# YufengJin/BundleSDF

Hardware: AMD Instinct MI355X
Metric: NeRF training rays/sec + ms/iter, 64-frame pool, 2048 rays/frame (higher is better)
Workload: dtype fp16 table+MLP (MFMA) / fp32 accumulate+Adam (amp)

## Files before the change

### bundlesdf_amd/csrc/field_step.hip

```cpp
#include <algorithm>
#include <cstdlib>
#include <cstring>
#include <array>
#include <type_traits>
#include <vector>

#include "nof_device.h"
#include "ray_trace.h"
#include "mlp_lds.h"

#pragma clang fp contract(off)

#ifndef NOF_ABLATE
#define NOF_ABLATE 0
#endif
#define ABL(bits) (NOF_ABLATE && (a.ablate & (bits)))
#define ABL_HOST(d, bits) (NOF_ABLATE && ((d)->ablate & (bits)))
#define ABL_SKIPQ(q) ((q) < 2 ? (1 << (23 + (q))) : (1 << (27 + (q))))

namespace nof {

typedef _Float16 h8v __attribute__((ext_vector_type(8)));
typedef float f16v __attribute__((ext_vector_type(16)));

constexpr int MLP_N_MAX = 9107 + 64 * 3;
struct MlpOff {
    int w1, b1, w2, b2, w3, b3, w4, b4, w5, b5, n, in, cin;
    __host__ __device__ MlpOff(int IN, int FF = 0) : in(IN), cin(24 + FF) {
        w1 = 0; b1 = 64 * IN; w2 = b1 + 64; b2 = w2 + 16 * 64; w3 = b2 + 16; b3 = w3 + 64 * cin; w4 = b3 + 64;
        b4 = w4 + 64 * 64; w5 = b4 + 64; b5 = w5 + 3 * 64; n = b5 + 3;
    }
};
constexpr int FR_L1 = 0, FR_L2 = 4, FR_L3 = 8, FR_L4 = 12, FR_L5 = 20, FR_B5 = 24, FR_B4 = 26, FR_B3 = 34,
              FR_B2 = 38, FR_B1 = 42, N_FRAGS = 46;
__device__ __forceinline__ int cin_col(int i, int ff) {
    return (i >= 1 && i <= 15) ? ff + 9 + i - 1
                               : ((i >= 16 && i <= 24) ? ff + i - 16 : ((i >= 25 && i < 25 + ff) ? i - 25 : -1));
}
constexpr float SH_C0 = 0.28209479177387814f, SH_C1 = 0.4886025119029199f;
constexpr float SH_C2_0 = 1.0925484305920792f, SH_C2_1 = -1.0925484305920792f, SH_C2_2 = 0.31539156525252005f,
                SH_C2_3 = -1.0925484305920792f, SH_C2_4 = 0.5462742152960396f;

struct FieldArgs {
    const float *rays;
    const float *tf;
    const float *intervals;
    const float *totals;
    float *rctx;
    const float *t_rand;
    uint32_t seed;
    int R, Kmax, N_oct, N_dep, S;
    int perturb;
    float near_sc, far_sc, trunc, ntr, lambda, fs_sdf, ffw, rgb_w, fs_w, empty_w, trunc_w;
    float fs_rgb_w;
    float inv_3R, inv_RS, inv_3RS;
    const float *loss_scale;
    const void *table;
    const float4 *levels;
    uint32_t L;
    int mlp_in;
    int n_ff;
    const float *ff;
    float *grad_ff;
    const void *frags;
    const float *bias;
    float *grad_table;
    __half *grad_table16;
    float *grad_mlp;
    float *ray_grad;
    uint32_t *tile_gmask;
    const uint4 *quads;
    uint32_t n_rows;
    bool quads_ready;
    float *loss_part;
    float *loss_acc;
    float *dbg_z;
    float *dbg_raw;
    uint8_t *dbg_valid;
    float *dbg_rgb;
    void *feat;
    void *dfeat;
    float *zbuf;
    uint8_t *tile_bwd;
    uint32_t slot_mask;
    int *tile_sid;
    int *n_tiles;
    float *ray_aux;
    float4 *tile_aux;
    int ablate;
    int xcd_order;
    const nof_step_params *sp;
    int no_dx;
    int scatter_lpw;
    float *rrec;
    int *ctile_list;
    int bwd_flush;
    int count_atomics;
    int compact_per;
    int encode_group;
};

constexpr int LOSS_ACC_COUNTERS = 136;
constexpr int LOSS_ACC_WORDS = 144;
constexpr int TREC = 12;
enum { TR_WSUM = 0, TR_NVALID, TR_LFS, TR_LEM, TR_LSDF, TR_CNT, TR_RACC = 8, TR_LFSR = 11 };
enum { TC_SIG = 1, TC_COL = 2, TC_CRCOL = 4, TC_CRSIG = 8 };
constexpr int LOSS_COPIES = 64, LOSS_SLOTS = 16, LOSS_FOLD_N = 13;
constexpr uint64_t LOSS_ZERO_WORDS = 16 + (uint64_t)LOSS_COPIES * LOSS_SLOTS;

__device__ __forceinline__ FieldArgs step_args(const FieldArgs &a0) {
    FieldArgs a = a0;
    if (a0.sp) {
        a.trunc = a0.sp->trunc;
        a.seed = a0.sp->seed;
    }
    return a;
}

__device__ __forceinline__ const FieldArgs &late_args() {
    auto k = __builtin_amdgcn_kernarg_segment_ptr();
    asm volatile("" : "+s"(k));
    return *(const FieldArgs *)k;
}

__device__ __forceinline__ int acc_row(int q, int h) { return (q & 3) + 8 * (q >> 2) + 4 * h; }

template <int CTRL, int ROWS = 0xf>
__device__ __forceinline__ float dpp_add(float v) {
    return v + __builtin_bit_cast(float, __builtin_amdgcn_update_dpp(0, __builtin_bit_cast(int, v), CTRL, ROWS, 0xf, true));
}
__device__ __forceinline__ float row_prefix(float v) {
    v = dpp_add<0x111>(v);
    v = dpp_add<0x112>(v);
    v = dpp_add<0x114>(v);
    return dpp_add<0x118>(v);
}
__device__ __forceinline__ float lane_value(float v, int l) {
    return __builtin_bit_cast(float, __builtin_amdgcn_readlane(__builtin_bit_cast(int, v), l));
}
__device__ __forceinline__ float wave_sum(float v) {
    v = row_prefix(v);
    v = dpp_add<0x142, 0xa>(v);
    v = dpp_add<0x143, 0xc>(v);
    return lane_value(v, 63);
}
__device__ __forceinline__ void half_sums(float v, float &s0, float &s1) {
    v = row_prefix(v);
    v = dpp_add<0x142, 0xa>(v);
    s0 = lane_value(v, 31);
    s1 = lane_value(v, 63);
}

__device__ __forceinline__ float sigmoidf(float x) { return __builtin_amdgcn_rcpf(1.0f + __expf(-x)); }
__device__ __forceinline__ int xcd_block(int b, int nb) {
    const int per = nb >> 3, rem = nb & 7, x = b & 7, i = b >> 3;
    return (x < rem ? x * (per + 1) : rem * (per + 1) + (x - rem) * per) + i;
}

__device__ __forceinline__ uint32_t hash32(uint32_t x) {
    x ^= x >> 16; x *= 0x7feb352dU; x ^= x >> 15; x *= 0x846ca68bU; x ^= x >> 16;
    return x;
}
__device__ __forceinline__ float rng_uniform(uint32_t seed, uint32_t ray, uint32_t s) {
    uint32_t h = hash32(seed ^ hash32(ray * 0x9E3779B1U + hash32(s + 0x632BE5ABU)));
    return (float)(h >> 8) * (1.0f / 16777216.0f);
}

__device__ __forceinline__ float linspace01(int i, int n) {
    if (n == 1) return 0.0f;
    const float step = 1.0f / (float)(n - 1);
    return (i < n / 2) ? __builtin_fmaf(step, (float)i, 0.0f) : __builtin_fmaf(-step, (float)(n - 1 - i), 1.0f);
}

template <typename TM> struct FragT;
template <> struct FragT<_Float16> { typedef h8v T; };
template <> struct FragT<float> { struct T { float v[8]; }; };

template <typename TM> __device__ __forceinline__ void frag_set(typename FragT<TM>::T &f, int j, float x);
template <> __device__ __forceinline__ void frag_set<_Float16>(h8v &f, int j, float x) { f[j] = (_Float16)x; }
template <> __device__ __forceinline__ void frag_set<float>(FragT<float>::T &f, int j, float x) { f.v[j] = x; }
template <typename TM> __device__ __forceinline__ float frag_get(const typename FragT<TM>::T &f, int j);
template <> __device__ __forceinline__ float frag_get<_Float16>(const h8v &f, int j) { return (float)f[j]; }
// ... 977 lines not shown
#pragma unroll
        for (int d = 0; d < 3; ++d) {
            pos[k][d] = __builtin_fmaf(x01[d], li.scale, 0.5f);
            pg[d] = (uint32_t)pos[k][d];
            pos[k][d] = __builtin_amdgcn_fractf(pos[k][d]);
        }
        base[k] = dense_base_v(li.off, pg, rs[k]);
    }
    typedef typename std::conditional<sizeof(TT) == 4, float4, uint2>::type Raw;
    Raw raw[G][4];
    const __amdgpu_buffer_rsrc_t trs = table_rsrc(a.table);
    if constexpr (sizeof(TT) == 2) {
        if (a.quads) {
            const __amdgpu_buffer_rsrc_t qrs = table_rsrc(a.quads);
#pragma unroll
            for (int k = 0; k < G; ++k) {
                const uint32_t b0 = dense[k] ? base[k] : 0u, b1 = dense[k] ? base[k] + rs2[k] : 0u;
                const u4v q0 = __builtin_amdgcn_raw_buffer_load_b128(qrs, b0 * 16u, 0, 0);
                const u4v q1 = __builtin_amdgcn_raw_buffer_load_b128(qrs, b1 * 16u, 0, 0);
                raw[k][0] = make_uint2(q0.x, q0.y);
                raw[k][1] = make_uint2(q0.z, q0.w);
                raw[k][2] = make_uint2(q1.x, q1.y);
                raw[k][3] = make_uint2(q1.z, q1.w);
            }
            goto sums;
        }
    }
#pragma unroll
    for (int k = 0; k < G; ++k)
#pragma unroll
        for (int i = 0; i < 4; ++i) {
            raw[k][i] = Raw{};
            if (dense[k]) {
                const uint32_t row = base[k] + ((i & 1) ? rs[k] : 0u) + ((i & 2) ? rs2[k] : 0u);
                if constexpr (sizeof(TT) == 4) {
                    const TT *ptr = tab + (size_t)row * 2;
                    typedef float f4a __attribute__((ext_vector_type(4), aligned(8)));
                    const f4a v = *reinterpret_cast<const f4a *>(ptr);
                    raw[k][i] = make_float4(v.x, v.y, v.z, v.w);
                } else {
                    raw[k][i] = table_pair16(trs, row);
                }
            }
        }
sums:
#pragma unroll
    for (int k = 0; k < G; ++k) {
        out[k][0] = 0.f;
        out[k][1] = 0.f;
        if (!(on && lvs[k] < (int)a.L)) continue;
        if (!dense[k]) {
            encode_level<TT>(a, lis[k], x01, out[k]);
            continue;
        }
        if constexpr (sizeof(TT) == 2) {
            float o0 = 0.f, o1 = 0.f;
#pragma unroll
            for (int idx = 0; idx < 8; ++idx) {
                float w = 1.f;
#pragma unroll
                for (int d = 0; d < 3; ++d) w *= ((idx >> d) & 1) ? pos[k][d] : 1 - pos[k][d];
                const uint32_t pr = (idx & 1) ? raw[k][idx >> 1].y : raw[k][idx >> 1].x;
                asm("v_fma_mix_f32 %0, %1, %2, %0 op_sel_hi:[0,1,0]" : "+v"(o0) : "v"(w), "v"(pr));
                asm("v_fma_mix_f32 %0, %1, %2, %0 op_sel:[0,1,0] op_sel_hi:[0,1,0]" : "+v"(o1) : "v"(w), "v"(pr));
            }
            out[k][0] = o0;
            out[k][1] = o1;
        } else {
            float e[8][2];
#pragma unroll
            for (int i = 0; i < 4; ++i) {
                e[2 * i][0] = raw[k][i].x; e[2 * i][1] = raw[k][i].y;
                e[2 * i + 1][0] = raw[k][i].z; e[2 * i + 1][1] = raw[k][i].w;
            }
#pragma unroll
            for (int idx = 0; idx < 8; ++idx) {
                float w = 1.f;
#pragma unroll
                for (int d = 0; d < 3; ++d) w *= ((idx >> d) & 1) ? pos[k][d] : 1 - pos[k][d];
                out[k][0] = __builtin_fmaf(w, e[idx][0], out[k][0]);
                out[k][1] = __builtin_fmaf(w, e[idx][1], out[k][1]);
            }
        }
    }
}

template <typename TM, typename TT, int G, bool DBG>
__global__ __launch_bounds__(512) __attribute__((amdgpu_num_sgpr(80),
                                                 amdgpu_waves_per_eu(sizeof(TM) == 2 ? (G == 1 ? 8 : G == 2 ? 6 : 4) : (G == 4 ? 4 : 5), 8)))
void k_encode(FieldArgs a_) {
    const FieldArgs a = step_args(a_);
    const int lane = threadIdx.x & 63, n = lane & 31, h = lane >> 5;
    const int ntiles = a.S / 32;
    constexpr int WPB = 8;
    extern __shared__ __attribute__((aligned(16))) char smem[];
    {
        typedef __attribute__((address_space(1))) void *GPtr;
        typedef __attribute__((address_space(3))) void *LPtr;
        const int wv = threadIdx.x >> 6;
        if (ABL(16)) {
            const uint4 *src = reinterpret_cast<const uint4 *>(a.frags);
            uint4 *dst = reinterpret_cast<uint4 *>(smem);
            for (int i = threadIdx.x; i < 8 * 64 * 8 * (int)sizeof(TM) / 16; i += blockDim.x) dst[i] = src[i];
            float *s_b = reinterpret_cast<float *>(smem + 8 * 64 * 8 * sizeof(TM));
            for (int i = threadIdx.x; i < 2 * 64; i += blockDim.x) s_b[i] = a.bias[i];
            __syncthreads();
        } else {
#pragma unroll
            for (int i = 0; i < (int)sizeof(TM) / 2; ++i) {
                const size_t off = (size_t)i * 8192 + (size_t)wv * 1024;
                __builtin_amdgcn_global_load_lds((GPtr)((const char *)a.frags + off + lane * 16), (LPtr)(smem + off), 16,
                                                 0, 0);
            }
            if (wv < 2)
                __builtin_amdgcn_global_load_lds((GPtr)(a.bias + wv * 64 + lane),
                                                 (LPtr)(smem + 8 * 64 * 8 * sizeof(TM) + wv * 256), 4, 0, 0);
        }
    }
    uint4 *lvt = reinterpret_cast<uint4 *>(smem + 8 * 64 * 8 * sizeof(TM) + 2 * 64 * sizeof(float)) + (threadIdx.x >> 6) * 32;
    level_table(a, lvt, lane);
    const int bx = (a.xcd_order & 1) ? xcd_block(blockIdx.x, gridDim.x) : (int)blockIdx.x;
    const int gw0 = __builtin_amdgcn_readfirstlane(bx * WPB + (int)(threadIdx.x >> 6));
    const bool in_range = gw0 < a.R * ntiles;
    const int gw = in_range ? gw0 : a.R * ntiles - 1;
    const int r = gw / ntiles, t = gw - r * ntiles;
    if (ABL(1 << 19)) return;
    const RayCtx c = load_ray(a, r);
    const int s = 32 * t + n;
    const size_t sid = (size_t)r * a.S + s;
    float z = sample_z(a, r, s, c.depth, c.vdepth, c.total, c.box);
    if (ABL(4)) {
        const float z2 = sample_z(a, r, s, c.depth * 0.999f, c.vdepth, c.total * 0.999f, c.box);
        z = z2 == 12345.f ? z2 : z;
    }
    float p[3], x[3];
    const bool valid = sample_point(c, z, p, x);
    if (h == 0 && in_range) {
        a.zbuf[sid] = z;
        if (DBG && a.dbg_z) a.dbg_z[sid] = z;
        if (DBG && a.dbg_valid) a.dbg_valid[sid] = valid;
    }
    if (ABL(8192)) return;
    const float x01[3] = {(x[0] + 1) / 2, (x[1] + 1) / 2, (x[2] + 1) / 2};
    typename FragT<TM>::T f[2];
#pragma unroll
    for (int g0 = 0; g0 < 8; g0 += G) {
        int lvs[G];
#pragma unroll
        for (int k = 0; k < G; ++k) lvs[k] = lane_level((g0 + k) >> 2, (g0 + k) & 3, h);
        float v[G][2];
        encode_levels<TT, G, true, true>(a, lvs, valid && !ABL(8), x01, v, lvt);
#pragma unroll
        for (int k = 0; k < G; ++k) {
            frag_set<TM>(f[(g0 + k) >> 2], 2 * ((g0 + k) & 3), v[k][0]);
            frag_set<TM>(f[(g0 + k) >> 2], 2 * ((g0 + k) & 3) + 1, v[k][1]);
        }
    }
    {
        if (!ABL(64)) __syncthreads();
        if (!in_range) return;
        const FieldArgs a = step_args(late_args());
        const bool tvalid = __any(valid);
        uint8_t *flag = a.tile_bwd + (size_t)r * ntiles + t;
        float4 *trec = reinterpret_cast<float4 *>(a.rrec + ((size_t)r * ntiles + t) * TREC);
        float ws = 0.f, nv = 0.f;
        if (!ABL(2)) half_sums(h == 0 ? bell_weight(a, c.depth, z) : (valid ? 1.f : 0.f), ws, nv);
        if (!tvalid && !(DBG && a.dbg_raw)) {
            if (lane == 0) {
                *flag = 0;
                if (trec) {
                    trec[0] = make_float4(ws, nv, 0.f, 0.f);
                    trec[1] = make_float4(0.f, 0.f, 0.f, 0.f);
                }
            }
            return;
        }
        const TM *s_fr = reinterpret_cast<const TM *>(smem);
        const float *s_b = reinterpret_cast<const float *>(smem + 8 * 64 * 8 * sizeof(TM));
        Acts<TM> A;
        A.X[0] = f[0];
        A.X[1] = f[1];
        float sdf = 0.f;
        f16v l2;
        if (ABL(256)) {
#pragma unroll
            for (int q = 0; q < 16; ++q) l2[q] = 0.f;
            sdf = z * 1e-3f;
        } else {
            mlp_sdf_net<TM>(LdsWt<TM>(s_fr, lane), s_b, A, lane, sdf, l2);
        }
        const float w = bell_weight(a, c.depth, z);
        const bool front = z < c.depth - a.trunc;
        const bool fsr = a.fs_rgb_w > 0.f && front && valid && c.rtype == 0;
        const bool colour = __any(w > 0.f && valid) || __any(fsr) || (DBG && a.dbg_raw != nullptr);
        const float sv = valid ? 1.f : 0.f;
        const bool back = z > c.depth + a.trunc * a.ntr;
        const float sdfm = (!front && !back && c.vdepth) ? 1.f : 0.f;
        const bool fsm = (c.depth > a.far_sc) && (sdf < a.fs_sdf);
        const bool em = front && (c.depth <= a.far_sc) && (sdf < 1.f);
        const float efs = fsm ? (sdf - a.fs_sdf) : 0.f;
        const float esdf = (z + sdf * a.trunc) * sdfm - c.depth * sdfm;
        float dsdf = a.fs_w * 0.5f * 2.f * efs * sv * a.inv_RS;
        dsdf += em ? a.fs_w * a.empty_w * (sdf > 1.f ? 1.f : (sdf < 1.f ? -1.f : 0.f)) * sv * a.inv_RS : 0.f;
        dsdf += a.trunc_w * 0.5f * 2.f * esdf * sdfm * a.trunc * sv * a.inv_RS;
        const bool cand = tvalid && c.rtype == 0 && (__any(w > 0.f && valid) || __any(dsdf != 0.f) || __any(fsr));
        if (lane == 0) *flag = cand ? (colour ? 1 : 2) : (colour ? 3 : 0);
        if (trec && !ABL(2)) {
            float lfs = 0.f, lem = 0.f, lsd = 0.f;
            if (__any(dsdf != 0.f)) {
                half_sums(h == 0 ? a.fs_w * 0.5f * efs * efs * sv * a.inv_RS
                                 : (em ? a.fs_w * a.empty_w * fabsf(sdf - 1.f) * sv * a.inv_RS : 0.f),
                          lfs, lem);
                float unused;
                half_sums(h == 0 ? a.trunc_w * 0.5f * esdf * esdf * sv * a.inv_RS : 0.f, lsd, unused);
            }
            if (lane == 0) {
                const int cnt = TC_SIG | (colour ? TC_COL : 0) | (cand ? (colour ? TC_CRCOL : TC_CRSIG) : 0);
                trec[0] = make_float4(ws, nv, lfs, lem);
                trec[1] = make_float4(lsd, __int_as_float(cnt), 0.f, 0.f);
            }
            if (DBG && a.dbg_raw && h == 0) a.dbg_raw[(((size_t)r * ntiles + t) * 32 + n) * 4 + 3] = sdf;
        }
        const size_t slot = (size_t)r * ntiles + t;
        if (ABL(32768)) return;
        if (cand) {
            store_chunk<TM>(a.feat, (size_t)r * a.S + 32 * t, n, 0, h, f[0]);
            store_chunk<TM>(a.feat, (size_t)r * a.S + 32 * t, n, 1, h, f[1]);
            if (h == 0) a.tile_aux[slot * TILE_AUX + 64 + n] = make_float4(dsdf, valid ? w : 0.f, sv, fsr ? 1.f : 0.f);
            const uint32_t gmask = (uint32_t)__ballot(h == 0 && valid && (w > 0.f || dsdf != 0.f || fsr));
            if (lane == 0) a.tile_gmask[slot] = gmask;
        }
        if (colour) {
            typename FragT<TM>::T cin;
            acc_to_frag<TM>(l2, 0, false, cin);
            store_cin<TM>(a.tile_aux + slot * TILE_AUX, lane, cin);
        }
    }
}

template <typename TM>
__device__ __forceinline__ void stage_mlp(const FieldArgs &a, char *smem) {
    TM *s_fr = reinterpret_cast<TM *>(smem);
    float *s_b = reinterpret_cast<float *>(smem + N_FRAGS * 64 * 8 * sizeof(TM));
    const uint4 *src = reinterpret_cast<const uint4 *>(a.frags);
// ... 803 lines not shown
}
}

namespace {
struct FieldWorkspace {
    size_t feat, dfeat, zbuf, tile_bwd, tile_sid, n_tiles, ray_aux, tile_aux, rctx, gmask, rrec, ctile, total;
    FieldWorkspace(int R, int S, int mlp_dtype) {
        auto al = [](size_t b) { return (b + 255) & ~(size_t)255; };
        const size_t el = mlp_dtype == NOF_F16 ? 2 : 4, n = (size_t)R * S, nt = (size_t)R * (S / 32);
        size_t o = 0;
        feat = o; o += al(n * 32 * el);
        dfeat = o; o += al(n * 32 * el);
        zbuf = o; o += al(n * 4);
        tile_bwd = o; o += al(nt);
        tile_sid = o; o += al(nt * 4);
        n_tiles = o; o += al(4 * nof::LOSS_ZERO_WORDS);
        ray_aux = o; o += al((size_t)R * nof::RAY_AUX * 4);
        tile_aux = o; o += al(nt * nof::TILE_AUX * 16);
        rctx = o; o += al((size_t)R * nof::RCTX * 4);
        gmask = o; o += al(nt * 4);
        rrec = o; o += al(nt * nof::TREC * 4);
        ctile = o; o += al(nt * 4);
        total = o;
    }
};
}

extern "C" size_t nof_field_workspace_bytes(int32_t R, int32_t S, int32_t mlp_dtype) {
    return FieldWorkspace(R, S, mlp_dtype).total;
}

extern "C" int nof_field_workspace_offsets(int32_t R, int32_t S, int32_t mlp_dtype, uint64_t *offsets, int32_t n) {
    if (R < 0 || S <= 0 || !offsets || n < NOF_WS_SECTIONS)
        return nof::set_error(NOF_EINVAL, "field_workspace_offsets: bad R=%d S=%d or n=%d < %d", R, S, n,
                              NOF_WS_SECTIONS);
    const FieldWorkspace w(R, S, mlp_dtype);
    const size_t o[NOF_WS_SECTIONS] = {w.feat, w.dfeat, w.zbuf, w.tile_bwd, w.tile_sid, w.n_tiles, w.ray_aux,
                                       w.tile_aux, w.rctx, w.gmask, w.rrec, w.ctile, w.total};
    for (int i = 0; i < NOF_WS_SECTIONS; ++i) offsets[i] = o[i];
    return NOF_OK;
}

namespace {
bool quads_on(const nof_field_desc *d) {
    return d->table_quads && d->table_rows > 0 && d->mlp_dtype == NOF_F16 && d->table_dtype == NOF_F16 &&
           d->R >= (d->quads_min_rays > 0 ? d->quads_min_rays : 32768) && !ABL_HOST(d, 512);
}
int cu_count() {
    int dev = 0, n_cu = 256;
    if (hipGetDevice(&dev) != hipSuccess ||
        hipDeviceGetAttribute(&n_cu, hipDeviceAttributeMultiprocessorCount, dev) != hipSuccess)
        n_cu = 256;
    return n_cu;
}
}

extern "C" size_t nof_field_desc_size(void) { return sizeof(nof_field_desc); }

extern "C" int nof_quad_mirror(const nof_field_desc *d, void *stream) {
    if (d->L > 16 || d->C != 2)
        return nof::set_error(NOF_EINVAL, "quad_mirror: needs C=2, L<=16 (got %u,%u)", d->C, d->L);
    if (d->R <= 0 || !quads_on(d)) return NOF_OK;
    nof::FieldArgs a{};
    a.table = d->table; a.levels = (const float4 *)d->levels; a.L = d->L;
    a.quads = (const uint4 *)d->table_quads; a.n_rows = (uint32_t)d->table_rows;
    const int n_cu = cu_count();
    hipLaunchKernelGGL(nof::k_quad_mirror, dim3((int)std::min<int64_t>((int64_t)n_cu * 8, nof::div_up(a.n_rows, 256))),
                       dim3(256), 0, (hipStream_t)stream, a);
    return nof::check_launch("quad_mirror");
}

extern "C" int nof_field_step(const nof_field_desc *d, void *stream) {
    if (d->S % 32 != 0 || d->S > 320 || d->N_oct + d->N_dep != d->S)
        return nof::set_error(NOF_EINVAL, "field_step: S=%d must be N_oct+N_dep, a multiple of 32, <= 320", d->S);
    if (d->L > 16 || d->C != 2 || d->D != 3)
        return nof::set_error(NOF_EINVAL, "field_step: needs D=3, C=2, L<=16 (got %u,%u,%u)", d->D, d->C, d->L);
    if (d->R <= 0) return NOF_OK;
    if (d->bwd_flush < 0 || d->bwd_flush > 2)
        return nof::set_error(NOF_EINVAL, "field_step: bwd_flush %d (0 by batch size, 1 per wave, 2 block)", d->bwd_flush);
    if (d->compact_per_block != 0 && (d->compact_per_block < 256 || d->compact_per_block > nof::COMPACT_PER_BLOCK ||
                                      d->compact_per_block % 256 != 0))
        return nof::set_error(NOF_EINVAL, "field_step: compact_per_block %d (0 by batch size, else a multiple of 256 "
                              "in [256, %d])", d->compact_per_block, nof::COMPACT_PER_BLOCK);
    if (d->encode_group != 0 && d->encode_group != 1 && d->encode_group != 2 && d->encode_group != 4)
        return nof::set_error(NOF_EINVAL, "field_step: encode_group %d (0 by batch size, or 1, 2, 4)", d->encode_group);
    if (d->n_ff < 0 || d->n_ff > 3 || (d->n_ff > 0 && (!d->ff || !d->grad_ff)))
        return nof::set_error(NOF_EINVAL, "field_step: frame_features must be 0..3 with ff and grad_ff set (got %d)",
                              d->n_ff);
    if (d->mlp_dtype == NOF_F16 && !d->grad_table16)
        return nof::set_error(NOF_EINVAL, "field_step: amp mode needs grad_table16 (fp16 table gradient)");
    if (d->ablate && !NOF_ABLATE)
        return nof::set_error(NOF_EINVAL, "field_step: ablate bits need a -DNOF_ABLATE=1 build (timing experiments only)");
    if (!d->workspace) return nof::set_error(NOF_EINVAL, "field_step: workspace is NULL (nof_field_workspace_bytes)");
    const int slots = d->scatter_slots ? d->scatter_slots : 512;
    if (slots < 64 || slots > 2048 || (slots & (slots - 1)))
        return nof::set_error(NOF_EINVAL, "field_step: scatter_slots must be a power of two in [64, 2048]");
    const bool amp = d->mlp_dtype == NOF_F16 && d->table_dtype == NOF_F16;
    if (!amp && !(d->mlp_dtype == NOF_F32 && d->table_dtype == NOF_F32))
        return nof::set_error(NOF_EINVAL, "field_step: mlp/table dtype must both be f16 (amp) or both f32");

    nof::FieldArgs a;
    a.rays = d->rays; a.tf = d->tf; a.intervals = d->intervals; a.totals = d->totals; a.t_rand = d->t_rand;
    a.seed = d->seed; a.R = d->R; a.Kmax = d->Kmax; a.N_oct = d->N_oct; a.N_dep = d->N_dep; a.S = d->S;
    a.perturb = d->perturb; a.near_sc = d->near_sc; a.far_sc = d->far_sc; a.trunc = d->trunc;
    a.ntr = d->neg_trunc_ratio; a.lambda = d->sdf_lambda; a.fs_sdf = d->fs_sdf; a.ffw = d->first_frame_weight;
    a.rgb_w = d->rgb_weight; a.fs_w = d->fs_weight; a.empty_w = d->empty_weight; a.trunc_w = d->trunc_weight;
    a.inv_3R = 1.0f / (3.0f * (float)d->R);
    a.inv_RS = 1.0f / ((float)d->R * (float)d->S);
    a.inv_3RS = 1.0f / (3.0f * (float)d->R * (float)d->S);
    a.xcd_order = d->xcd_order;
    a.no_dx = d->skip_pose_grad != 0;
    a.quads = quads_on(d) ? (const uint4 *)d->table_quads : nullptr;
    a.n_rows = (uint32_t)d->table_rows;
    a.quads_ready = d->quads_prebuilt != 0;
    {
        const int L = std::max(1, (int)d->L);
        const int want = d->R >= 196608 ? 16 : (d->R >= 32768 ? 8 : (d->R >= 8192 ? 4 : 2));
        a.scatter_lpw = std::max(1, std::min(L, d->scatter_levels_per_wave > 0 ? (int)d->scatter_levels_per_wave : want));
    }
    a.bwd_flush = d->bwd_flush;
    a.count_atomics = d->count_atomics != 0;
    a.compact_per = d->compact_per_block;
    a.encode_group = d->encode_group ? d->encode_group : (d->R >= 8192 ? 1 : nof::ENCODE_GROUP_SMALL);
    a.sp = d->step_params;
    a.fs_rgb_w = d->fs_rgb_weight;
    a.loss_scale = d->loss_scale; a.table = d->table; a.levels = (const float4 *)d->levels; a.L = d->L;
    a.mlp_in = (int)(d->L * d->C);
    a.n_ff = d->n_ff; a.ff = d->ff; a.grad_ff = d->grad_ff;
    a.frags = d->frags; a.bias = d->bias; a.grad_table = d->grad_table; a.grad_mlp = d->grad_mlp;
    a.grad_table16 = (__half *)d->grad_table16;
    a.ray_grad = d->ray_grad; a.loss_acc = d->loss_acc; a.dbg_z = d->dbg_z; a.dbg_raw = d->dbg_raw;
    a.dbg_valid = d->dbg_valid; a.dbg_rgb = d->dbg_rgb; a.ablate = d->ablate;
    a.slot_mask = (uint32_t)slots - 1;
    {
        char *w = (char *)d->workspace;
        const FieldWorkspace ws(d->R, d->S, d->mlp_dtype);
        a.feat = w + ws.feat;
        a.dfeat = w + ws.dfeat;
        a.zbuf = (float *)(w + ws.zbuf);
        a.tile_bwd = (uint8_t *)(w + ws.tile_bwd);
        a.tile_sid = (int *)(w + ws.tile_sid);
        a.n_tiles = (int *)(w + ws.n_tiles);
        a.loss_part = (float *)(w + ws.n_tiles) + 16;
        a.ray_aux = (float *)(w + ws.ray_aux);
        a.tile_aux = (float4 *)(w + ws.tile_aux);
        a.rctx = (float *)(w + ws.rctx);
        a.tile_gmask = (uint32_t *)(w + ws.gmask);
        a.rrec = (float *)(w + ws.rrec);
        a.ctile_list = (int *)(w + ws.ctile);
    }

    hipStream_t st = (hipStream_t)stream;
    const int n_cu = cu_count();
    return amp ? launch_field<_Float16, __half, 4>(a, n_cu, st) : launch_field<float, float, 4>(a, n_cu, st);
}

extern "C" int nof_field_timing(int32_t enable) {
    g_timing.on = enable != 0;
    g_timing.used = 0;
    return NOF_OK;
}

extern "C" int nof_field_timing_collect(float *ms_sum, int32_t n, int32_t *calls) {
    if (!ms_sum || n < N_FIELD_KERNELS) return nof::set_error(NOF_EINVAL, "field_timing_collect: need 4 floats");
    for (int k = 0; k < n; ++k) ms_sum[k] = 0.f;
    for (size_t i = 0; i < g_timing.used; ++i) {
        auto &e = g_timing.sets[i];
        if (hipEventSynchronize(e[N_FIELD_KERNELS]) != hipSuccess)
            return nof::set_error(NOF_ELAUNCH, "field_timing_collect: event sync failed");
        for (int k = 0; k < N_FIELD_KERNELS; ++k) {
            float ms = 0.f;
            if (hipEventElapsedTime(&ms, e[k], e[k + 1]) != hipSuccess)
                return nof::set_error(NOF_ELAUNCH, "field_timing_collect: elapsed time failed");
            ms_sum[k] += ms;
        }
    }
    if (calls) *calls = (int32_t)g_timing.used;
    g_timing.used = 0;
    return NOF_OK;
}

extern "C" int nof_query_sdf(const void *table, int32_t table_dtype, const float *level_table, uint32_t L,
                             const void *frags, const float *bias, int32_t mlp_dtype, int32_t mlp_in,
                             const float *points, int64_t n, const float *gx, const float *gy, const float *gz,
                             int32_t nx, int32_t ny, int32_t nz, const uint8_t *occ, int32_t occ_n, float *sdf,
                             void *stream) {
    if (!table || !level_table || !frags || !bias || !sdf || L == 0 || L > 16 || mlp_in != (int)L * 2)
        return nof::set_error(NOF_EINVAL, "query_sdf: bad table / MLP arguments (C = 2, L <= 16)");
    if (table_dtype != mlp_dtype) return nof::set_error(NOF_EINVAL, "query_sdf: table and MLP dtypes must match");
    if (!points && (!gx || !gy || !gz || nx <= 0 || ny <= 0 || nz <= 0))
        return nof::set_error(NOF_EINVAL, "query_sdf: need points or three grid axes");
    if (!points) n = (int64_t)nx * ny * nz;
    if (n <= 0) return NOF_OK;
    nof::FieldArgs a{};
    a.table = table;
    a.levels = reinterpret_cast<const float4 *>(level_table);
    a.L = L;
    a.mlp_in = mlp_in;
    a.frags = frags;
    a.bias = bias;
    nof::QueryArgs q{points, gx, gy, gz, nx, ny, nz, n, occ, occ_n, sdf};
    hipStream_t st = (hipStream_t)stream;
    const int n_cu = cu_count();
    const int64_t ntile = (n + 31) / 32;
    const int blocks = (int)std::min<int64_t>((ntile + 3) / 4, (int64_t)n_cu * 2);
    if (mlp_dtype == NOF_F16) {
// ... 216 lines not shown
```

### bundlesdf_amd/fused.py

```python
import ctypes
import dataclasses
import math
import os

import numpy as np
import torch

from . import _lib
from . import exchange as EX
from . import mlp_layout as ML

_F32, _F16 = 0, 1
MAX_LEVEL_RES = 1023
QUADS_MIN_RAYS = 32768


def lr_at(cfg, global_step, base):
    n_iters = cfg["n_step"] + 1
    if global_step <= 10:
        return base
    last = 10 * ((global_step - 1) // 10)
    return base * (cfg["decay_rate"] ** (float(last) / n_iters))


def truncation(cfg, global_step):
    kind = cfg.get("trunc_decay_type", "") or ""
    if kind == "linear":
        t = cfg["trunc_start"] - (cfg["trunc_start"] - cfg["trunc"]) * float(global_step) / cfg["n_step"]
    elif kind == "exp":
        lamb = np.log(cfg["trunc"] / cfg["trunc_start"]) / (cfg["n_step"] / 4)
        t = max(cfg["trunc_start"] * np.exp(global_step * lamb), cfg["trunc"])
    elif kind == "":
        t = cfg["trunc"]
    else:
        raise NotImplementedError(f"trunc_decay_type {kind!r} (the reference knows '', 'linear', 'exp')")
    return float(t) * cfg["sc_factor"]


allreduce_gradients = EX.allreduce_mean


class _HipOps:

    def __init__(self, fs):
        self.fs = fs

    def grad16_to_f32(self, src16, dst32, n):
        _lib.check(_lib.lib().nof_grad16_to_f32(_lib.ptr(src16), _lib.ptr(dst32), n, _lib.stream_of(dst32)),
                   "grad16_to_f32")

    def unscale_check(self, g, n, f16_lo=0, f16_hi=0):
        fs = self.fs
        _lib.check(_lib.lib().nof_unscale_check(_lib.ptr(g), n, _lib.ptr(fs.scale), _lib.ptr(fs.found_inf), None, 0,
                                                f16_lo, f16_hi, _lib.stream_of(g)), "unscale")

    def check16(self, g16, n):
        fs = self.fs
        _lib.check(_lib.lib().nof_unscale_check(None, 0, _lib.ptr(fs.scale), _lib.ptr(fs.found_inf), _lib.ptr(g16), n,
                                                0, 0, _lib.stream_of(g16)), "check16")

    def adam(self, p, g, m, v, n, group1_start, mirror, sp, g16=None, active=None):
        fs = self.fs
        lr0 = lr_at(fs.cfg, fs.global_step, fs.cfg["lrate"])
        lr1 = lr_at(fs.cfg, fs.global_step, fs.cfg["lrate_pose"])
        mn = 0 if mirror is None else int(mirror.numel())
        _lib.check(_lib.lib().nof_adam_step(_lib.ptr(p), _lib.ptr(g), _lib.ptr(m), _lib.ptr(v), n, group1_start, lr0, lr1,
                                            0.9, 0.999, 1e-15, _lib.ptr(fs.adam_t), _lib.ptr(fs.found_inf),
                                            _lib.ptr(mirror), mn, _lib.ptr(g16), _lib.ptr(fs.scale),
                                            _lib.ctypes.c_void_p(sp), _lib.ptr(active), _lib.stream_of(p)), "adam")

    @staticmethod
    def active_flags(n, dev):
        return torch.zeros(int(_lib.lib().nof_adam_active_bytes(n)), dtype=torch.uint8, device=dev)

    def scaler_update(self):
        fs = self.fs
        _lib.check(_lib.lib().nof_scaler_update(_lib.ptr(fs.scale), _lib.ptr(fs.tracker), _lib.ptr(fs.found_inf),
                                                _lib.ptr(fs.adam_t), 2.0, 0.5, fs.growth_interval,
                                                1 if fs.amp else 0, _lib.stream_of(fs.scale)), "scaler")


@dataclasses.dataclass(slots=True)
class Knobs:
    ablate: int = 0
    scatter_slots: int = 0
    scatter_levels_per_wave: int = 0
    bwd_flush: int = 0
    compact_per_block: int = 0
    encode_group: int = 0
    quads_min_rays: int = 0
    count_atomics: bool = False
    xcd_order: int = dataclasses.field(default_factory=lambda: int(os.environ.get("NOF_XCD_ORDER", "1")))
    use_quads: bool = True
    quad_fork: bool = dataclasses.field(default_factory=lambda: os.environ.get("NOF_QUAD_FORK", "1") != "0")

    DESCRIPTOR = ("ablate", "scatter_slots", "scatter_levels_per_wave", "bwd_flush", "compact_per_block",
                  "encode_group", "quads_min_rays", "count_atomics", "xcd_order")


class FusedStep:
    def __init__(self, cfg, pool, c2w, occ, grid, mlp, pose_array, amp=None, frame_start=None, blocks_per_cu=0,
                 process_group=None, world_size=1, time_kernels=False, feature_array=None, exchange=None):
        dev = pool.device
        if dev.type != "cuda":
            raise RuntimeError("FusedStep needs a HIP device (no CPU fallback)")
        _lib.lib()
        self.cfg, self.dev = cfg, dev
        self.amp = bool(cfg["amp"] if amp is None else amp)
        self.pool = pool.contiguous().float()
        self.c2w = c2w.to(dev).float().contiguous()
        self.F = self.c2w.shape[0]
        self.occ = occ.to(dev).to(torch.uint8).contiguous()
        self.Nocc = int(self.occ.shape[0])
        self.Kmax = 3 * self.Nocc
        self.grid, self.mlp, self.pose_array = grid, mlp, pose_array
        self.L, self.C = grid.n_levels, grid.level_dim
        self.n_in = self.L * self.C
        assert self.C == 2 and self.n_in <= 32, "fused path: C=2, L<=16"
        self.knobs = Knobs()
        self.frame_start = None
        if frame_start is not None:
            fst = np.asarray(frame_start, np.int64).ravel()
            if fst.size < 2 or fst[0] != 0 or (np.diff(fst) <= 0).any() or fst[-1] > self.pool.shape[0]:
                raise ValueError("frame_start must be an increasing prefix [0, ..., <= N_pool] with no empty frame")
            self.frame_start = torch.as_tensor(fst, dtype=torch.int64, device=dev)
        emb = grid.embeddings.data.reshape(-1)
        sd = dict(mlp.named_parameters())
        mlp_flat = torch.cat([sd[k].data.reshape(-1).float() for k in ML.MLP_KEYS])
        self.feature_array = feature_array
        self.n_ff = 0 if feature_array is None else int(feature_array.data.shape[1])
        if not 0 <= self.n_ff <= 3:
            raise ValueError(f"fused path: frame_features must be <= 3 (got {self.n_ff})")
        assert mlp_flat.numel() == ML.offsets(self.n_in, self.n_ff)[1]
        pose = pose_array.data.data.reshape(-1)
        feat = (torch.zeros(0) if feature_array is None else feature_array.data.data.reshape(-1).float())
        if feature_array is not None and feature_array.data.shape[0] != self.F:
            raise ValueError("feature_array rows must match the number of frames")
        self.n_emb, self.n_mlp, self.n_pose = emb.numel(), mlp_flat.numel(), pose.numel()
        self.n_feat = feat.numel()
        self.P = torch.cat([emb.to(dev), mlp_flat.to(dev), feat.to(dev), pose.to(dev)]).contiguous()
        self.mlp_off = self.n_emb
        self.feat_off = self.n_emb + self.n_mlp
        self.pose_off = self.feat_off + self.n_feat
        grid.embeddings.data = self.P[:self.n_emb].view(-1, self.C)
        o = self.mlp_off
        for k in ML.MLP_KEYS:
            n = sd[k].numel()
            sd[k].data = self.P[o:o + n].view(sd[k].shape)
            o += n
        pose_array.data.data = self.P[self.pose_off:].view(self.F, 6)
        if feature_array is not None:
            feature_array.data.data = self.P[self.feat_off:self.pose_off].view(self.F, self.n_ff)
        self.Gbuf = torch.zeros(self.P.numel() + 1, dtype=torch.float32, device=dev)
        self.G = self.Gbuf[:self.P.numel()]
        self.M = torch.zeros_like(self.P)
        self.V = torch.zeros_like(self.P)
        self.adam_active = _HipOps.active_flags(self.P.numel(), dev)
        self.emb16 = torch.empty(self.n_emb, dtype=torch.float16, device=dev) if self.amp else None
        self.G16 = torch.zeros(self.n_emb, dtype=torch.float16, device=dev) if self.amp else None
        self.quads = torch.empty(self.n_emb * 2, dtype=torch.int32, device=dev) if self.amp else None
        self._side = torch.cuda.Stream(dev) if self.amp else None
        if self.amp:
# ... 100 lines not shown
            self.adam_t.zero_()
            self.step_dev.zero_()
        self.global_step = 0
        self._step_dev_at = 0

    def _alloc(self, R):
        if self._R == R:
            return
        d = self.dev
        self.rays = torch.empty(R, 12, device=d)
        self.intervals = torch.empty(R, self.Kmax, 2, device=d)
        self.totals = torch.empty(R, device=d)
        self.counts = torch.empty(R, dtype=torch.int32, device=d)
        self.ray_grad = torch.empty(R, 12, device=d)
        self.ids = torch.empty(R, dtype=torch.int32, device=d)
        S = self.cfg["N_samples"] + self.cfg["N_samples_around_depth"]
        nbytes = _lib.lib().nof_field_workspace_bytes(R, S, _F16 if self.amp else _F32)
        self.workspace = torch.empty(nbytes, dtype=torch.uint8, device=d)
        self._R = R
        self._graphs = None

    def sample_ids(self, rays_per_frame, seed):
        nf = int(self.frame_start.numel()) - 1
        R = nf * rays_per_frame
        self._alloc(R)
        _lib.check(_lib.lib().nof_sample_batch(_lib.ptr(self.frame_start), nf, rays_per_frame, seed & 0xFFFFFFFF,
                                               _lib.ptr(self.ids), None, _lib.stream_of(self.ids)), "sample_batch")
        return self.ids

    def step(self, ids=None, t_rand=None, debug=False, seed=None, perturb=True, grad_hook=None):
        if ids is None:
            raise ValueError("step(ids=...) or sample_ids() first")
        ids = ids.to(self.dev).to(torch.int32).contiguous()
        R = ids.numel()
        self._alloc(R)
        if ids.data_ptr() != self.ids.data_ptr():
            self.ids.copy_(ids)
        dbg = self._field_part(R, None, t_rand, debug, seed, perturb)
        if grad_hook is not None:
            grad_hook(self)
        grads = self._exchange_and_optimize(debug)
        self.global_step += 1
        out = {"loss_terms": self.loss_acc[:8], "fs_rgb_loss": self.loss_acc[140]}
        if debug:
            out.update(dbg=dbg, grads=grads)
        return out

    def _prologue(self, sched=None):
        L = _lib.lib()
        sd = None if sched is None else _lib.ctypes.byref(sched)
        _lib.check(L.nof_step_prologue(sd, _lib.ptr(self.step_dev) if sched is not None else None,
                                       _lib.ptr(self.step_params) if sched is not None else None,
                                       _lib.ctypes.c_void_p(self.P.data_ptr() + 4 * self.pose_off), _lib.ptr(self.c2w),
                                       self.F, float(self.pose_array.max_trans),
                                       float(self.pose_array.max_rot / 180.0 * math.pi), _lib.ptr(self.tf_buf),
                                       _lib.ptr(self.pose_jac),
                                       _lib.ctypes.c_void_p(self.P.data_ptr() + 4 * self.mlp_off),
                                       _lib.ptr(self.pack_idx), self.n_frag_elems, 5 * 64, _lib.ptr(self.frags),
                                       _lib.ptr(self.bias), _F16 if self.amp else _F32, _lib.stream_of(self.P)),
                   "step_prologue")

    def _trace(self, R, sp):
        cfg = self.cfg
        sc = cfg["sc_factor"]
        perm = getattr(self, "_trace_perm", None)
        if perm is not None and sp is not None:
            _lib.check(_lib.lib().nof_trace_rays_epoch(
                _lib.ptr(self.pool), _lib.ptr(perm), _lib.ptr(self.epoch_step0), R, _lib.ptr(self.tf_buf),
                _lib.ptr(self.occ), self.Nocc, self.Kmax, cfg["near"] * sc, cfg["far"] * sc,
                truncation(cfg, self.global_step), _lib.ptr(self.rays), _lib.ptr(self.intervals),
                _lib.ptr(self.totals), _lib.ptr(self.counts), _lib.ctypes.c_void_p(sp), _lib.stream_of(self.P)),
                "trace_rays_epoch")
            return
        _lib.check(_lib.lib().nof_trace_rays(_lib.ptr(self.pool), _lib.ptr(self.ids), R, _lib.ptr(self.tf_buf),
                                             _lib.ptr(self.occ), self.Nocc, self.Kmax, cfg["near"] * sc,
                                             cfg["far"] * sc, truncation(cfg, self.global_step), _lib.ptr(self.rays),
                                             _lib.ptr(self.intervals), _lib.ptr(self.totals), _lib.ptr(self.counts),
                                             _lib.ctypes.c_void_p(sp), _lib.stream_of(self.P)), "trace_rays")

    def wait_exchange(self):
        if self.ex is not None:
            self.ex.wait_mirror()

    def _uses_quads(self):
        return self.quads is not None and self.knobs.use_quads

    def _field_desc(self, R):
        D = _lib.FieldDesc()
        D.R, D.L, D.C, D.D = R, self.L, self.C, 3
        D.table = (self.emb16 if self.amp else self.P).data_ptr()
        D.levels = self.levels.data_ptr()
        D.table_dtype = D.mlp_dtype = _F16 if self.amp else _F32
        if self._uses_quads():
            D.table_quads, D.table_rows = self.quads.data_ptr(), self.n_emb // 2
        for k in Knobs.DESCRIPTOR:
            setattr(D, k, int(getattr(self.knobs, k)))
        return D

    def _fork_quad_mirror(self, R):
        if (not self._uses_quads() or not self.knobs.quad_fork or self.time_kernels or R == 0
                or (self.ex is not None and self.exchange == "sharded")):
            return None
        if R < (self.knobs.quads_min_rays or QUADS_MIN_RAYS):
            return None
        D = self._field_desc(R)
        main = torch.cuda.current_stream(self.dev)
        self._side.wait_stream(main)
        with torch.cuda.stream(self._side):
            _lib.check(_lib.lib().nof_quad_mirror(_lib.ctypes.byref(D), _lib.stream_of(self.P)), "quad_mirror")
        return lambda: main.wait_stream(self._side)

    def _field_part(self, R, sp, t_rand=None, debug=False, seed=None, perturb=True, prologue=True, trace=True,
                    join_quads=None):
        cfg = self.cfg
        L = _lib.lib()
        st = _lib.stream_of(self.P)
        sc = cfg["sc_factor"]
        trunc = truncation(cfg, self.global_step)
        S = cfg["N_samples"] + cfg["N_samples_around_depth"]
        if prologue:
            if join_quads is None:
                join_quads = self._fork_quad_mirror(R)
            self._prologue()
        if trace:
            self._trace(R, sp)
        if not self._capturing:
            self.wait_exchange()
        if join_quads is not None:
            join_quads()
        if R == 0:
            self.loss_acc.zero_()
        dbg = None
        if debug:
            dbg = dict(z=torch.zeros(R, S, device=self.dev), raw=torch.zeros(R, S, 4, device=self.dev),
                       valid=torch.zeros(R, S, dtype=torch.uint8, device=self.dev),
                       rgb=torch.zeros(R, 3, device=self.dev))
        D = self._field_desc(R)
        D.rays, D.tf, D.intervals, D.totals = self.rays.data_ptr(), self.tf_buf.data_ptr(), \
            self.intervals.data_ptr(), self.totals.data_ptr()
        if t_rand is not None:
            t_rand = t_rand.to(self.dev).float().contiguous()
            self._t_rand = t_rand
            D.t_rand = t_rand.data_ptr()
        D.seed = (self.global_step * 0x9E3779B1 + (0 if seed is None else seed)) & 0xFFFFFFFF
        D.Kmax, D.N_oct, D.N_dep, D.S = self.Kmax, cfg["N_samples"], cfg["N_samples_around_depth"], S
        D.perturb = 1 if perturb else 0
        D.near_sc, D.far_sc, D.trunc = cfg["near"] * sc, cfg["far"] * sc, trunc
        D.neg_trunc_ratio, D.sdf_lambda, D.fs_sdf = cfg["neg_trunc_ratio"], cfg["sdf_lambda"], cfg["fs_sdf"]
        D.first_frame_weight, D.rgb_weight, D.fs_weight = cfg["first_frame_weight"], cfg["rgb_weight"], cfg["fs_weight"]
        D.empty_weight, D.trunc_weight = cfg["empty_weight"], cfg["trunc_weight"]
        D.fs_rgb_weight = float(cfg.get("fs_rgb_weight", 0) or 0)
        D.loss_scale = self.scale.data_ptr()
        D.frags, D.bias = self.frags.data_ptr(), self.bias.data_ptr()
        D.grad_table, D.grad_mlp = self.G.data_ptr(), self.G.data_ptr() + 4 * self.mlp_off
        D.grad_table16 = self.G16.data_ptr() if self.amp else None
        D.ray_grad, D.loss_acc = self.ray_grad.data_ptr(), self.loss_acc.data_ptr()
        if dbg is not None:
            D.dbg_z, D.dbg_raw, D.dbg_valid, D.dbg_rgb = (dbg["z"].data_ptr(), dbg["raw"].data_ptr(),
                                                          dbg["valid"].data_ptr(), dbg["rgb"].data_ptr())
        D.workspace = self.workspace.data_ptr()
        D.step_params = sp
        D.skip_pose_grad = 0 if self.pose_grad else 1
        if debug or self.time_kernels:
            D.count_atomics = 1
        if self._uses_quads():
            D.quads_prebuilt = 0 if join_quads is None else 1
# ... 450 lines not shown
```

### include/nof.h

```cpp
#ifndef NOF_H
#define NOF_H

#include <stddef.h>
#include <stdint.h>

#ifdef __cplusplus
extern "C" {
#endif

typedef enum {
    NOF_OK = 0,
    NOF_EINVAL = 1,
    NOF_ELAUNCH = 2,
    NOF_EDEVICE = 3
} nof_status;

typedef enum { NOF_F32 = 0, NOF_F16 = 1 } nof_dtype;

#define NOF_MAX_LEVELS 32

const char *nof_last_error(void);
const char *nof_version(void);


int nof_grid_encode_forward(const float *inputs, const void *embeddings, const int32_t *offsets, void *outputs,
                            uint32_t B, uint32_t D, uint32_t C, uint32_t L, float S, uint32_t H,
                            int calc_grad_inputs, void *dy_dx, uint32_t gridtype, int align_corners,
                            int dtype, void *stream);

int nof_grid_encode_backward(const void *grad, const float *inputs, const void *embeddings,
                             const int32_t *offsets, void *grad_embeddings, uint32_t B, uint32_t D, uint32_t C,
                             uint32_t L, float S, uint32_t H, int calc_grad_inputs, const void *dy_dx,
                             void *grad_inputs, uint32_t gridtype, int align_corners, int dtype, void *stream);

int nof_sample_rays_uniform_occupied_voxels(const float *z_in_out, const float *z_sampled, float *z_vals,
                                            int32_t n_rays, int32_t n_intersect, int32_t n_samples,
                                            int32_t *error_count, void *stream);

int nof_postprocess_octree_ray_tracing(const int64_t *ray_index, const float *depth_in_out,
                                       const int64_t *unique_intersect_ray_ids, const int64_t *start_poss,
                                       int64_t n_hits, int64_t n_unique, int32_t max_intersections,
                                       float *out, void *stream);

int nof_ray_color_to_texture_uv(const int64_t *F, const float *V, const float *hit_locations,
                                const int64_t *hit_face_ids, const float *uvs_tex, float *uvs, int64_t n_hits,
                                void *stream);


void nof_level_params(uint32_t L, float S, uint32_t H, float *scales, uint32_t *resolutions);

int nof_octree_ray_trace(const uint8_t *occ, int32_t N, const float *rays_o, const float *rays_d, int32_t R,
                         int32_t Kmax, float *out, int32_t *counts, void *stream);

typedef struct {
    double lr0, lr1;
    float trunc;
    uint32_t seed;
    uint32_t batch_seed;
    int32_t step;
} nof_step_params;

typedef struct {
    double lrate, lrate_pose, decay_rate;
    double trunc, trunc_start, sc_factor;
    int32_t trunc_decay;
    int32_t n_step;
    uint32_t seed_base, batch_seed_base;
} nof_schedule_desc;

int nof_step_schedule(const nof_schedule_desc *d, int32_t *step, nof_step_params *out, void *stream);

int nof_trace_rays(const float *pool, const int32_t *ids, int32_t R, const float *tf, const uint8_t *occ, int32_t N,
                   int32_t Kmax, float near_sc, float far_sc, float trunc, float *rays_out, float *intervals,
                   float *totals, int32_t *counts, const nof_step_params *sp, void *stream);

int nof_trace_rays_epoch(const float *pool, const int32_t *perm, const int32_t *epoch_step0, int32_t R,
                         const float *tf, const uint8_t *occ, int32_t N, int32_t Kmax, float near_sc, float far_sc,
                         float trunc, float *rays_out, float *intervals, float *totals, int32_t *counts,
                         const nof_step_params *sp, void *stream);

int nof_sample_batch(const int64_t *frame_start, int32_t F, int32_t rays_per_frame, uint32_t seed, int32_t *ids,
                     const nof_step_params *sp, void *stream);

int nof_pack_mlp(const float *mlp, const int32_t *idx, int32_t n_frag_elems, int32_t n_bias, void *frags,
                 float *bias, int mlp_dtype, void *stream);

typedef struct {
    const float *rays;
    const float *tf;
    const float *intervals;
    const float *totals;
    const float *t_rand;
    uint32_t seed;
    int32_t R, Kmax, N_oct, N_dep, S, perturb;
    float near_sc, far_sc, trunc, neg_trunc_ratio, sdf_lambda, fs_sdf, first_frame_weight;
    float rgb_weight, fs_weight, empty_weight, trunc_weight;
    float fs_rgb_weight;
    int32_t skip_pose_grad;
    const float *loss_scale;
    const nof_step_params *step_params;
    const void *table;
    const float *levels;
// ... 233 lines not shown
```

Baseline: 29.81 million.

## Add lean encode tail for tiles with only free-space samples

Adds a specialized tail to the encode kernel for tiles whose samples all lie in front of the truncation band or on far rays, with no free-space RGB term. These tiles only need the SDF net output and the free-space/empty loss gradients, so the tail skips the colour branch and the general loss bookkeeping. It is on by default and can be switched off with a flag bit folded into encode_group. The risk is a loss or gradient mismatch with the general path, plus extra code size and register pressure in the encode kernel.

```diff
diff --git a/bundlesdf_amd/csrc/field_step.hip b/bundlesdf_amd/csrc/field_step.hip
--- a/bundlesdf_amd/csrc/field_step.hip
+++ b/bundlesdf_amd/csrc/field_step.hip
@@ -98,6 +98,7 @@
     int count_atomics;
     int compact_per;
     int encode_group;
+    int encode_front;
 };
 
 constexpr int LOSS_ACC_COUNTERS = 136;
@@ -1241,6 +1242,72 @@
                 out[k][1] = __builtin_fmaf(w, e[idx][1], out[k][1]);
             }
         }
+    }
+}
+
+__device__ __forceinline__ bool front_only_tile(const FieldArgs &a, const RayCtx &c, float z, bool valid) {
+    const bool front = z < c.depth - a.trunc;
+    const float dz = z - c.depth;
+    const bool band = (dz <= a.trunc * a.ntr) && (dz >= -a.trunc);
+    const bool fsr = a.fs_rgb_w > 0.f && front && valid && c.rtype == 0;
+    return !__any(!((c.depth > a.far_sc) || (front && !band)) || fsr);
+}
+
+template <typename TM>
+__device__ __forceinline__ void encode_front_tail(const FieldArgs &a, const RayCtx &c, const char *smem, int r, int t, int ntiles,
+                                                  bool valid, const typename FragT<TM>::T (&f)[2]) {
+    const int lane = threadIdx.x & 63, n = lane & 31, h = lane >> 5;
+    const bool tvalid = __any(valid);
+    const size_t slot = (size_t)r * ntiles + t;
+    uint8_t *flag = a.tile_bwd + slot;
+    float4 *trec = reinterpret_cast<float4 *>(a.rrec + slot * TREC);
+    const float sv = valid ? 1.f : 0.f;
+    float ws = 0.f, nv = 0.f;
+    if (!ABL(2)) half_sums(h == 0 ? 0.f : sv, ws, nv);
+    if (!tvalid) {
+        if (lane == 0) {
+            *flag = 0;
+            if (trec) {
+                trec[0] = make_float4(ws, nv, 0.f, 0.f);
+                trec[1] = make_float4(0.f, 0.f, 0.f, 0.f);
+            }
+        }
+        return;
+    }
+    const TM *s_fr = reinterpret_cast<const TM *>(smem);
+    const float *s_b = reinterpret_cast<const float *>(smem + 8 * 64 * 8 * sizeof(TM));
+    Acts<TM> A;
+    A.X[0] = f[0];
+    A.X[1] = f[1];
+    float sdf = 0.f;
+    f16v l2;
+    mlp_sdf_net<TM>(LdsWt<TM>(s_fr, lane), s_b, A, lane, sdf, l2);
+    const bool far = c.depth > a.far_sc;
+    const bool fsm = far && (sdf < a.fs_sdf);
+    const bool em = !far && (sdf < 1.f);
+    const float efs = fsm ? (sdf - a.fs_sdf) : 0.f;
+    float dsdf = a.fs_w * 0.5f * 2.f * efs * sv * a.inv_RS;
+    dsdf += em ? a.fs_w * a.empty_w * (sdf > 1.f ? 1.f : (sdf < 1.f ? -1.f : 0.f)) * sv * a.inv_RS : 0.f;
+    const bool cand = c.rtype == 0 && __any(dsdf != 0.f);
+    if (lane == 0) *flag = cand ? 2 : 0;
+    if (trec && !ABL(2)) {
+        float lfs = 0.f, lem = 0.f;
+        if (__any(dsdf != 0.f))
+            half_sums(h == 0 ? a.fs_w * 0.5f * efs * efs * sv * a.inv_RS
+                             : (em ? a.fs_w * a.empty_w * fabsf(sdf - 1.f) * sv * a.inv_RS : 0.f),
+                      lfs, lem);
+        if (lane == 0) {
+            trec[0] = make_float4(ws, nv, lfs, lem);
+            trec[1] = make_float4(0.f, __int_as_float(TC_SIG | (cand ? TC_CRSIG : 0)), 0.f, 0.f);
+        }
+    }
+    if (ABL(32768)) return;
+    if (cand) {
+        store_chunk<TM>(a.feat, (size_t)r * a.S + 32 * t, n, 0, h, f[0]);
+        store_chunk<TM>(a.feat, (size_t)r * a.S + 32 * t, n, 1, h, f[1]);
+        if (h == 0) a.tile_aux[slot * TILE_AUX + 64 + n] = make_float4(dsdf, 0.f, sv, 0.f);
+        const uint32_t gmask = (uint32_t)__ballot(h == 0 && valid && dsdf != 0.f);
+        if (lane == 0) a.tile_gmask[slot] = gmask;
     }
 }
 
@@ -1301,6 +1368,7 @@
     }
     if (ABL(8192)) return;
     const float x01[3] = {(x[0] + 1) / 2, (x[1] + 1) / 2, (x[2] + 1) / 2};
+    const bool lean = !DBG && a.encode_front && front_only_tile(a, c, z, valid);
     typename FragT<TM>::T f[2];
 #pragma unroll
     for (int g0 = 0; g0 < 8; g0 += G) {
@@ -1319,6 +1387,10 @@
         if (!ABL(64)) __syncthreads();
         if (!in_range) return;
         const FieldArgs a = step_args(late_args());
+        if (lean) {
+            encode_front_tail<TM>(a, c, smem, r, t, ntiles, valid, f);
+            return;
+        }
         const bool tvalid = __any(valid);
         uint8_t *flag = a.tile_bwd + (size_t)r * ntiles + t;
         float4 *trec = reinterpret_cast<float4 *>(a.rrec + ((size_t)r * ntiles + t) * TREC);
@@ -2288,8 +2360,10 @@
                                       d->compact_per_block % 256 != 0))
         return nof::set_error(NOF_EINVAL, "field_step: compact_per_block %d (0 by batch size, else a multiple of 256 "
                               "in [256, %d])", d->compact_per_block, nof::COMPACT_PER_BLOCK);
-    if (d->encode_group != 0 && d->encode_group != 1 && d->encode_group != 2 && d->encode_group != 4)
-        return nof::set_error(NOF_EINVAL, "field_step: encode_group %d (0 by batch size, or 1, 2, 4)", d->encode_group);
+    const int egroup = d->encode_group & ~NOF_ENCODE_GENERAL;
+    if (egroup != 0 && egroup != 1 && egroup != 2 && egroup != 4)
+        return nof::set_error(NOF_EINVAL, "field_step: encode_group %d (0 by batch size, or 1, 2, 4; + %d: no front-only path)",
+                              d->encode_group, NOF_ENCODE_GENERAL);
     if (d->n_ff < 0 || d->n_ff > 3 || (d->n_ff > 0 && (!d->ff || !d->grad_ff)))
         return nof::set_error(NOF_EINVAL, "field_step: frame_features must be 0..3 with ff and grad_ff set (got %d)",
                               d->n_ff);
@@ -2327,7 +2401,8 @@
     a.bwd_flush = d->bwd_flush;
     a.count_atomics = d->count_atomics != 0;
     a.compact_per = d->compact_per_block;
-    a.encode_group = d->encode_group ? d->encode_group : (d->R >= 8192 ? 1 : nof::ENCODE_GROUP_SMALL);
+    a.encode_group = egroup ? egroup : (d->R >= 8192 ? 1 : nof::ENCODE_GROUP_SMALL);
+    a.encode_front = (d->encode_group & NOF_ENCODE_GENERAL) ? 0 : 1;
     a.sp = d->step_params;
     a.fs_rgb_w = d->fs_rgb_weight;
     a.loss_scale = d->loss_scale; a.table = d->table; a.levels = (const float4 *)d->levels; a.L = d->L;
diff --git a/bundlesdf_amd/fused.py b/bundlesdf_amd/fused.py
--- a/bundlesdf_amd/fused.py
+++ b/bundlesdf_amd/fused.py
@@ -78,6 +78,9 @@
         _lib.check(_lib.lib().nof_scaler_update(_lib.ptr(fs.scale), _lib.ptr(fs.tracker), _lib.ptr(fs.found_inf),
                                                 _lib.ptr(fs.adam_t), 2.0, 0.5, fs.growth_interval,
                                                 1 if fs.amp else 0, _lib.stream_of(fs.scale)), "scaler")
+
+
+ENCODE_GENERAL = 8
 
 
 @dataclasses.dataclass(slots=True)
@@ -344,6 +347,15 @@
         if self.ex is not None:
             self.ex.wait_mirror()
 
+    @property
+    def encode_front_path(self):
+        return not (self.knobs.encode_group & ENCODE_GENERAL)
+
+    @encode_front_path.setter
+    def encode_front_path(self, on):
+        g = self.knobs.encode_group & ~ENCODE_GENERAL
+        self.knobs.encode_group = g if on else g | ENCODE_GENERAL
+
     def _uses_quads(self):
         return self.quads is not None and self.knobs.use_quads
 
diff --git a/include/nof.h b/include/nof.h
--- a/include/nof.h
+++ b/include/nof.h
@@ -18,6 +18,7 @@
 typedef enum { NOF_F32 = 0, NOF_F16 = 1 } nof_dtype;
 
 #define NOF_MAX_LEVELS 32
+#define NOF_ENCODE_GENERAL 8
 
 const char *nof_last_error(void);
 const char *nof_version(void);
```

Result: slower. 29.34 million (-1.6%).
